# ZhaoyangLyu/Point_Diffusion_Refinement

Hardware: AMD Instinct MI355X
Metric: DDPM reverse steps/sec (T=1000, N=2048) (higher is better)
Workload: dtype f32; 1 GPU; BASELINE configs[1]: B=32/GPU, N=2048, 3072-pt mirrored condition, T=1000 DDPM reverse sampling, random-init dual-path PointNet++ (9.76 M params), cached condition step; global_batch=32, parallelism=dp1, launch=hipGraph replay, noise=device Philox, execution=fused channel-last HIP

## Files before the change

### point_diffusion_refinement_amd/csrc/abi.hip

```cpp
#include "pdr_common.h"

#include <atomic>
#include <cstring>

namespace {
thread_local char g_last_error[256] = "";

struct OptRow {
  const char* name;
  int def, lo, hi;
};
const OptRow k_opts[pdr::OPT_COUNT] = {
    {"fused_ws", 1, 0, 1},
    {"narrow_kc32", 1, 0, 1},
    {"fps_wave", 1, 0, 2},
    {"fps_lean", 1, 0, 1},
    {"knn_wave", 1, 0, 1},
    {"gn_fold_small", 1, 0, 1},
    {"ws_narrow3", 1, 0, 1},
    {"ws_xcd_order", 1, 0, 2},
    {"deep_chunks", 1, 0, 1},
    {"deep_ks", 1, 0, 1},
    {"deep_jobs32", 256, 0, 65536},
    {"deep_jobs64", 512, 0, 65536},
};
std::atomic<int> g_opts[pdr::OPT_COUNT];
std::atomic<bool> g_opts_init{false};

void opts_init() {
  if (!g_opts_init.load(std::memory_order_acquire)) {
    for (int i = 0; i < pdr::OPT_COUNT; ++i) g_opts[i].store(k_opts[i].def, std::memory_order_relaxed);
    g_opts_init.store(true, std::memory_order_release);
  }
}

int opt_index(const char* name) {
  if (!name) return -1;
  for (int i = 0; i < pdr::OPT_COUNT; ++i)
    if (std::strcmp(name, k_opts[i].name) == 0) return i;
  return -1;
}
}

namespace pdr {
void set_last_error(hipError_t e) {
  const char* s = hipGetErrorString(e);
  int i = 0;
  for (; s && s[i] && i < 255; ++i) g_last_error[i] = s[i];
  g_last_error[i] = 0;
}
int option(Opt o) {
  opts_init();
  return g_opts[o].load(std::memory_order_relaxed);
}
}

extern "C" int pdr_set_option(const char* name, int value) {
  const int i = opt_index(name);
  if (i < 0 || value < k_opts[i].lo || value > k_opts[i].hi) return PDR_EINVAL;
  opts_init();
  g_opts[i].store(value, std::memory_order_relaxed);
  return PDR_OK;
}

extern "C" int pdr_get_option(const char* name, int* value) {
  const int i = opt_index(name);
  if (i < 0 || !value) return PDR_EINVAL;
  *value = pdr::option(static_cast<pdr::Opt>(i));
  return PDR_OK;
}

extern "C" const char* pdr_option_name(int index) {
  return (index >= 0 && index < pdr::OPT_COUNT) ? k_opts[index].name : nullptr;
}

extern "C" int pdr_version(void) { return 200;  }
extern "C" const char* pdr_last_error(void) { return g_last_error; }
```

### point_diffusion_refinement_amd/csrc/fps.hip

```cpp
#include "pdr_common.h"

#include <cstdlib>

namespace {

constexpr int kMaxResidentN = 16384;

template <int T, int PPT>
__global__ __launch_bounds__(T) void fps_resident_kernel(
    const float* __restrict__ xyz, int N, int m, int R, int Rbits, int Q,
    int* __restrict__ idxs) {
  extern __shared__ __attribute__((aligned(16))) float smem[];
  constexpr int W = T / 64;
  float* sx = smem;
  float* sy = smem + N;
  float* sz = smem + 2 * N;
  unsigned long long* slots =
      reinterpret_cast<unsigned long long*>(smem + ((3 * N + 3) & ~3));

  const int b = blockIdx.x;
  const int tid = threadIdx.x;
  const float* p = xyz + static_cast<size_t>(b) * N * 3;
  int* out = idxs + static_cast<size_t>(b) * m;

  for (int i = tid; i < N; i += T) {
    sx[i] = p[i * 3 + 0];
    sy[i] = p[i * 3 + 1];
    sz[i] = p[i * 3 + 2];
  }

  float px[PPT], py[PPT], pz[PPT], tmp[PPT];
  unsigned low[PPT];
#pragma unroll
  for (int i = 0; i < PPT; ++i) {
    const int k = tid + i * T;
    if (k < N) {
      px[i] = p[k * 3 + 0];
      py[i] = p[k * 3 + 1];
      pz[i] = p[k * 3 + 2];
      const float mag = PDR_SUM3(px[i], py[i], pz[i]);
      tmp[i] = (static_cast<double>(mag) <= 1e-3) ? -1.0f : 1e10f;
      const unsigned rank = pdr::bitrev(static_cast<unsigned>(k % R), Rbits) * Q + k / R;
      low[i] = ((0xFFFFu - rank) << 16) | static_cast<unsigned>(k);
    } else {
      px[i] = py[i] = pz[i] = 0.0f;
      tmp[i] = -1.0f;
      low[i] = 0u;
    }
  }
#pragma unroll
  for (int a = 0; a < PPT - 1; ++a) {
#pragma unroll
    for (int c = 0; c < PPT - 1 - a; ++c) {
      if (low[c] < low[c + 1]) {
        float t;
        unsigned u;
        t = px[c]; px[c] = px[c + 1]; px[c + 1] = t;
        t = py[c]; py[c] = py[c + 1]; py[c + 1] = t;
        t = pz[c]; pz[c] = pz[c + 1]; pz[c + 1] = t;
        t = tmp[c]; tmp[c] = tmp[c + 1]; tmp[c + 1] = t;
        u = low[c]; low[c] = low[c + 1]; low[c + 1] = u;
      }
    }
  }

  if (tid == 0) out[0] = 0;
  __syncthreads();

  int old = 0;
  for (int j = 1; j < m; ++j) {
    const float x1 = sx[old], y1 = sy[old], z1 = sz[old];
    float best = -1.0f;
    unsigned bestlow = 0u;
#pragma unroll
    for (int i = 0; i < PPT; ++i) {
      const float dx = px[i] - x1, dy = py[i] - y1, dz = pz[i] - z1;
      const float d = PDR_SUM3(dx, dy, dz);
      const float d2 = fminf(d, tmp[i]);
      tmp[i] = d2;
      const bool gt = d2 > best;
      best = gt ? d2 : best;
      bestlow = gt ? low[i] : bestlow;
    }
    unsigned long long key =
        best < 0.0f ? 0ull : pdr::u64_from(__float_as_uint(best), bestlow);
    key = pdr::wave_max_u64(key);
    if constexpr (W > 1) {
      unsigned long long* s = slots + (j & 1) * W;
      if ((tid & 63) == 0) s[tid >> 6] = key;
      __syncthreads();
      unsigned long long r = s[0];
#pragma unroll
      for (int w = 1; w < W; ++w) {
        const unsigned long long o = s[w];
        r = o > r ? o : r;
      }
      key = r;
    }
    old = static_cast<int>(key & 0xFFFFull);
    if (tid == 0) out[j] = old;
  }
}

typedef float fps_f2 __attribute__((ext_vector_type(2)));

__device__ __forceinline__ void fps_combine(float& da, unsigned& la, float db, unsigned lb) {
  asm volatile(
      "v_cmp_gt_f32 vcc, %2, %0\n\t"
      "s_nop 1\n\t"
      "v_cndmask_b32 %0, %0, %2, vcc\n\t"
      "v_cndmask_b32 %1, %1, %3, vcc"
      : "+v"(da), "+v"(la)
      : "v"(db), "v"(lb)
      : "vcc");
}
__device__ __forceinline__ void fps_combine2(float& da, unsigned& la, float db, unsigned lb, float& dc,
                                             unsigned& lc, float dd, unsigned ld) {
  unsigned long long m;
  asm volatile(
      "v_cmp_gt_f32 vcc, %5, %0\n\t"
      "v_cmp_gt_f32 %4, %7, %2\n\t"
      "s_nop 0\n\t"
      "v_cndmask_b32 %0, %0, %5, vcc\n\t"
      "v_cndmask_b32 %1, %1, %6, vcc\n\t"
      "v_cndmask_b32 %2, %2, %7, %4\n\t"
      "v_cndmask_b32 %3, %3, %8, %4"
      : "+v"(da), "+v"(la), "+v"(dc), "+v"(lc), "=&s"(m)
      : "v"(db), "v"(lb), "v"(dd), "v"(ld)
      : "vcc");
}

template <int H>
__device__ __forceinline__ void fps_first2(const fps_f2& a, const fps_f2& b, float& bd0, unsigned& bs0, float& bd1,
                                           unsigned& bs1) {
  unsigned long long m;
  asm volatile(
      "v_cmp_gt_f32 vcc, %6, %5\n\t"
      "v_cmp_gt_f32 %4, %8, %7\n\t"
      "s_nop 0\n\t"
      "v_cndmask_b32 %0, %5, %6, vcc\n\t"
      "v_cndmask_b32 %1, %9, %10, vcc\n\t"
      "v_cndmask_b32 %2, %7, %8, %4\n\t"
      "v_cndmask_b32 %3, %11, %12, %4"
      : "=&v"(bd0), "=&v"(bs0), "=&v"(bd1), "=&v"(bs1), "=&s"(m)
      : "v"(a[0]), "v"(a[1]), "v"(b[0]), "v"(b[1]), "n"(2 * H), "n"(2 * H + 1), "n"(2 * H + 2), "n"(2 * H + 3)
      : "vcc");
}
template <int H>
__device__ __forceinline__ void fps_first1(const fps_f2& a, float& bd0, unsigned& bs0) {
  asm volatile(
      "v_cmp_gt_f32 vcc, %3, %2\n\t"
      "s_nop 1\n\t"
      "v_cndmask_b32 %0, %2, %3, vcc\n\t"
      "v_cndmask_b32 %1, %4, %5, vcc"
      : "=&v"(bd0), "=&v"(bs0)
      : "v"(a[0]), "v"(a[1]), "n"(2 * H), "n"(2 * H + 1)
      : "vcc");
}
template <int H, int NH>
__device__ __forceinline__ void fps_level0(const fps_f2 (&tmp)[NH], float (&bd)[NH], unsigned (&bs)[NH]) {
  if constexpr (H + 1 < NH) {
    fps_first2<H>(tmp[H], tmp[H + 1], bd[H], bs[H], bd[H + 1], bs[H + 1]);
    fps_level0<H + 2, NH>(tmp, bd, bs);
  } else if constexpr (H < NH) {
    fps_first1<H>(tmp[H], bd[H], bs[H]);
  }
}

template <int T, int PPT>
__global__ __launch_bounds__(T) void fps_wave_kernel(const float* __restrict__ xyz, int N, int m, int R,
                                                     int Rbits, int Q, int* __restrict__ idxs) {
  static_assert(PPT % 2 == 0, "points are processed in pairs");
  constexpr int W = T / 64;
  extern __shared__ __attribute__((aligned(16))) float4 cloud4[];
  __shared__ unsigned long long slots[2][W > 1 ? W : 1];
  const int b = blockIdx.x;
  const int lane = threadIdx.x;
  const float* p = xyz + static_cast<size_t>(b) * N * 3;
  int* out = idxs + static_cast<size_t>(b) * m;
  for (int i = lane; i < N; i += T) cloud4[i] = make_float4(p[i * 3 + 0], p[i * 3 + 1], p[i * 3 + 2], 0.0f);

  fps_f2 px[PPT / 2], py[PPT / 2], pz[PPT / 2], tmp[PPT / 2];
#pragma unroll
  for (int i = 0; i < PPT; ++i) {
    const int r = i * T + lane;
    const int hi = r / Q, lo = r - hi * Q;
    const int k = lo * R + static_cast<int>(pdr::bitrev(static_cast<unsigned>(hi), Rbits));
    const bool valid = hi < R && k < N;
    const int kk = valid ? k : 0;
    const float x = p[kk * 3 + 0], y = p[kk * 3 + 1], z = p[kk * 3 + 2];
    const float mag = PDR_SUM3(x, y, z);
    const float t0 = (!valid || static_cast<double>(mag) <= 1e-3) ? -1.0f : 1e10f;
    px[i >> 1][i & 1] = valid ? x : 0.0f;
    py[i >> 1][i & 1] = valid ? y : 0.0f;
    pz[i >> 1][i & 1] = valid ? z : 0.0f;
    tmp[i >> 1][i & 1] = t0;
  }
  if (lane == 0) out[0] = 0;
  __syncthreads();

  int old = 0;
  for (int j = 1; j < m; ++j) {
    const float4 c = cloud4[old];
    constexpr int G = (PPT / 2) < 8 ? (PPT / 2) : 8;
#pragma unroll
    for (int h0 = 0; h0 < PPT / 2; h0 += G) {
      fps_f2 dx[G], dy[G], dz[G], d[G];
#pragma unroll
      for (int g = 0; g < G; ++g) dy[g] = py[h0 + g] - c.y;
#pragma unroll
      for (int g = 0; g < G; ++g) dx[g] = px[h0 + g] - c.x;
#pragma unroll
      for (int g = 0; g < G; ++g) d[g] = dy[g] * dy[g];
#pragma unroll
      for (int g = 0; g < G; ++g) dz[g] = pz[h0 + g] - c.z;
#pragma unroll
      for (int g = 0; g < G; ++g) d[g] = __builtin_elementwise_fma(dx[g], dx[g], d[g]);
#pragma unroll
      for (int g = 0; g < G; ++g) d[g] = __builtin_elementwise_fma(dz[g], dz[g], d[g]);
#pragma unroll
      for (int g = 0; g < G; ++g) {
        fps_f2 r;
        asm("v_min_f32 %0, %1, %2" : "=v"(r[0]) : "v"(d[g][0]), "v"(tmp[h0 + g][0]));
        asm("v_min_f32 %0, %1, %2" : "=v"(r[1]) : "v"(d[g][1]), "v"(tmp[h0 + g][1]));
        tmp[h0 + g] = r;
      }
    }
    float bd[PPT / 2];
    unsigned bs[PPT / 2];
    fps_level0<0, PPT / 2>(tmp, bd, bs);
#pragma unroll
    for (int st = 1; st < PPT / 2; st <<= 1) {
#pragma unroll
      for (int i = 0; i + st < PPT / 2; i += 4 * st) {
        if (i + 3 * st < PPT / 2) fps_combine2(bd[i], bs[i], bd[i + st], bs[i + st], bd[i + 2 * st], bs[i + 2 * st],
                                               bd[i + 3 * st], bs[i + 3 * st]);
        else fps_combine(bd[i], bs[i], bd[i + st], bs[i + st]);
      }
    }
    const float best = bd[0];
    const unsigned vb = best < 0.0f ? 0u : __float_as_uint(best);
    const unsigned vmax = pdr::wave_max_u32(vb);
    const unsigned rk = 0xFFFFu - (bs[0] * static_cast<unsigned>(T) + static_cast<unsigned>(lane));
    const unsigned cand = (vb == vmax && best >= 0.0f) ? rk : 0u;
    unsigned win = pdr::wave_max_u32(cand);
    if constexpr (W > 1) {
      unsigned long long* sl = slots[j & 1];
      if ((lane & 63) == 0) sl[lane >> 6] = pdr::u64_from(vmax, win);
      __syncthreads();
      unsigned long long key = sl[0];
#pragma unroll
      for (int w = 1; w < W; ++w) {
        const unsigned long long o = sl[w];
        key = o > key ? o : key;
      }
      win = static_cast<unsigned>(key & 0xFFFFFFFFull);
    }
    const int rw = 0xFFFF - static_cast<int>(win);
    const int hw = rw / Q, lw = rw - hw * Q;
    old = win == 0u ? 0 : lw * R + static_cast<int>(pdr::bitrev(static_cast<unsigned>(hw), Rbits));
    if (lane == 0) out[j] = old;
  }
}

template <int T, int PPT>
int launch_wave(const float* xyz, int B, int N, int m, int R, int Rbits, int Q, int* idx, hipStream_t s) {
  hipLaunchKernelGGL((fps_wave_kernel<T, PPT>), dim3(B), dim3(T), static_cast<size_t>(N) * sizeof(float4), s, xyz, N,
                     m, R, Rbits, Q, idx);
  return pdr::check_launch();
}

__device__ __forceinline__ unsigned fps_wave_max_u32(unsigned v) {
  asm volatile(
      "s_nop 1\n\t"
      "v_max_u32_dpp %0, %0, %0 row_shr:1 row_mask:0xf bank_mask:0xf\n\t"
      "s_nop 1\n\t"
      "v_max_u32_dpp %0, %0, %0 row_shr:2 row_mask:0xf bank_mask:0xf\n\t"
      "s_nop 1\n\t"
      "v_max_u32_dpp %0, %0, %0 row_shr:4 row_mask:0xf bank_mask:0xf\n\t"
      "s_nop 1\n\t"
      "v_max_u32_dpp %0, %0, %0 row_shr:8 row_mask:0xf bank_mask:0xf\n\t"
      "s_nop 1\n\t"
      "v_max_u32_dpp %0, %0, %0 row_bcast:15 row_mask:0xa bank_mask:0xf\n\t"
      "s_nop 1\n\t"
      "v_max_u32_dpp %0, %0, %0 row_bcast:31 row_mask:0xc bank_mask:0xf\n\t"
      "s_nop 1"
      : "+v"(v));
  return __builtin_amdgcn_readlane(v, 63);
}

template <int T, int PPT>
__global__ __launch_bounds__(T) void fps_lean_kernel(const float* __restrict__ xyz, int N, int m, int R, int Rbits,
                                                     int Q, int* __restrict__ idxs) {
  static_assert(PPT % 2 == 0, "points are updated in pairs");
  constexpr int W = T / 64;
  extern __shared__ __attribute__((aligned(16))) float4 lean_cloud[];
  __shared__ unsigned long long slots[2][W > 1 ? W : 1];
  const int b = blockIdx.x;
  const int tid = threadIdx.x;
  const float* p = xyz + static_cast<size_t>(b) * N * 3;
  int* out = idxs + static_cast<size_t>(b) * m;
  for (int i = tid; i < N; i += T) lean_cloud[i] = make_float4(p[i * 3 + 0], p[i * 3 + 1], p[i * 3 + 2], 0.0f);

  float sx[PPT], sy[PPT], sz[PPT], st[PPT];
  unsigned low[PPT];
#pragma unroll
  for (int i = 0; i < PPT; ++i) {
    const int k = tid + i * T;
    if (k < N) {
      sx[i] = p[k * 3 + 0];
      sy[i] = p[k * 3 + 1];
      sz[i] = p[k * 3 + 2];
      const float mag = PDR_SUM3(sx[i], sy[i], sz[i]);
      st[i] = (static_cast<double>(mag) <= 1e-3) ? -1.0f : 1e10f;
      const unsigned rank = pdr::bitrev(static_cast<unsigned>(k % R), Rbits) * Q + k / R;
      low[i] = ((0xFFFFu - rank) << 16) | static_cast<unsigned>(k);
    } else {
      sx[i] = sy[i] = sz[i] = 0.0f;
      st[i] = -1.0f;
      low[i] = 0u;
    }
  }
#pragma unroll
  for (int a = 0; a < PPT - 1; ++a) {
#pragma unroll
    for (int c = 0; c < PPT - 1 - a; ++c) {
      if (low[c] < low[c + 1]) {
        float t;
        unsigned u;
        t = sx[c]; sx[c] = sx[c + 1]; sx[c + 1] = t;
        t = sy[c]; sy[c] = sy[c + 1]; sy[c + 1] = t;
        t = sz[c]; sz[c] = sz[c + 1]; sz[c + 1] = t;
        t = st[c]; st[c] = st[c + 1]; st[c + 1] = t;
        u = low[c]; low[c] = low[c + 1]; low[c + 1] = u;
      }
    }
  }
  fps_f2 px[PPT / 2], py[PPT / 2], pz[PPT / 2], tmp[PPT / 2];
#pragma unroll
  for (int i = 0; i < PPT; ++i) {
    px[i >> 1][i & 1] = sx[i];
    py[i >> 1][i & 1] = sy[i];
    pz[i >> 1][i & 1] = sz[i];
    tmp[i >> 1][i & 1] = st[i];
  }
  if (tid == 0) out[0] = 0;
  __syncthreads();

  int old = 0;
  for (int j = 1; j < m; ++j) {
    const float4 c = lean_cloud[old];
    constexpr int G = PPT / 2;
    fps_f2 dx[G], dy[G], dz[G], d[G];
#pragma unroll
    for (int g = 0; g < G; ++g) dy[g] = py[g] - c.y;
#pragma unroll
    for (int g = 0; g < G; ++g) dx[g] = px[g] - c.x;
#pragma unroll
    for (int g = 0; g < G; ++g) d[g] = dy[g] * dy[g];
#pragma unroll
    for (int g = 0; g < G; ++g) dz[g] = pz[g] - c.z;
#pragma unroll
    for (int g = 0; g < G; ++g) d[g] = __builtin_elementwise_fma(dx[g], dx[g], d[g]);
#pragma unroll
    for (int g = 0; g < G; ++g) d[g] = __builtin_elementwise_fma(dz[g], dz[g], d[g]);
    float best = -1.0f;
    unsigned bestlow = 0u;
#pragma unroll
    for (int g = 0; g < G; ++g) {
      fps_f2 r;
      asm("v_min_f32 %0, %1, %2" : "=v"(r[0]) : "v"(d[g][0]), "v"(tmp[g][0]));
      asm("v_min_f32 %0, %1, %2" : "=v"(r[1]) : "v"(d[g][1]), "v"(tmp[g][1]));
      tmp[g] = r;
#pragma unroll
      for (int e = 0; e < 2; ++e) {
        const bool gt = r[e] > best;
        best = gt ? r[e] : best;
        bestlow = gt ? low[2 * g + e] : bestlow;
      }
    }
    const unsigned vb = best < 0.0f ? 0u : __float_as_uint(best);
    const unsigned vmax = fps_wave_max_u32(vb);
    const unsigned cand = (vb == vmax && !(best < 0.0f)) ? bestlow : 0u;
    unsigned wlow = fps_wave_max_u32(cand);
    unsigned long long key = pdr::u64_from(vmax, wlow);
    if constexpr (W > 1) {
      unsigned long long* sl = slots[j & 1];
      if ((tid & 63) == 0) sl[tid >> 6] = key;
      __syncthreads();
      unsigned long long r = sl[0];
#pragma unroll
      for (int w = 1; w < W; ++w) {
        const unsigned long long o = sl[w];
        r = o > r ? o : r;
      }
      key = r;
    }
    old = static_cast<int>(key & 0xFFFFull);
    if (tid == 0) out[j] = old;
  }
}

template <int T, int PPT>
int launch_lean(const float* xyz, int B, int N, int m, int R, int Rbits, int Q, int* idx, hipStream_t s) {
  hipLaunchKernelGGL((fps_lean_kernel<T, PPT>), dim3(B), dim3(T), static_cast<size_t>(N) * sizeof(float4), s, xyz, N, m,
                     R, Rbits, Q, idx);
  return pdr::check_launch();
}

__global__ __launch_bounds__(1024) void fps_stream_kernel(
    const float* __restrict__ xyz, int N, int m, int R, int Rbits, int Q,
    float* __restrict__ temp, int* __restrict__ idxs) {
  __shared__ float sval[16];
  __shared__ unsigned long long srank[16];
  __shared__ int sold;
  const int b = blockIdx.x, tid = threadIdx.x;
  const float* p = xyz + static_cast<size_t>(b) * N * 3;
  float* tp = temp + static_cast<size_t>(b) * N;
  int* out = idxs + static_cast<size_t>(b) * m;
  for (int k = tid; k < N; k += 1024) {
    const float mag = PDR_SUM3(p[k * 3], p[k * 3 + 1], p[k * 3 + 2]);
    tp[k] = (static_cast<double>(mag) <= 1e-3) ? -1.0f : 1e10f;
  }
  if (tid == 0) out[0] = 0;
  __syncthreads();
  int old = 0;
  for (int j = 1; j < m; ++j) {
    const float x1 = p[old * 3], y1 = p[old * 3 + 1], z1 = p[old * 3 + 2];
    float best = -1.0f;
    unsigned long long bestrank = ~0ull;
    for (int k = tid; k < N; k += 1024) {
      const float dx = p[k * 3] - x1, dy = p[k * 3 + 1] - y1, dz = p[k * 3 + 2] - z1;
      const float d2 = fminf(PDR_SUM3(dx, dy, dz), tp[k]);
      tp[k] = d2;
      const unsigned long long rank =
          (static_cast<unsigned long long>(pdr::bitrev(k % R, Rbits)) * Q + k / R) << 32 |
          static_cast<unsigned>(k);
      const bool better = d2 > best || (d2 == best && d2 >= 0.0f && rank < bestrank);
      best = better ? d2 : best;
      bestrank = better ? rank : bestrank;
    }
#pragma unroll
    for (int off = 32; off >= 1; off >>= 1) {
      const float ov = __shfl_xor(best, off, 64);
      const unsigned long long orank = __shfl_xor(bestrank, off, 64);
      const bool better = ov > best || (ov == best && orank < bestrank);
      best = better ? ov : best;
      bestrank = better ? orank : bestrank;
    }
    if ((tid & 63) == 0) {
      sval[tid >> 6] = best;
      srank[tid >> 6] = bestrank;
    }
    __syncthreads();
    if (tid == 0) {
      float bv = sval[0];
      unsigned long long br = srank[0];
      for (int w = 1; w < 16; ++w) {
        const bool better = sval[w] > bv || (sval[w] == bv && srank[w] < br);
        bv = better ? sval[w] : bv;
        br = better ? srank[w] : br;
      }
      sold = bv < 0.0f ? 0 : static_cast<int>(br & 0xFFFFFFFFull);
      out[j] = sold;
    }
    __syncthreads();
    old = sold;
  }
}

template <int T, int PPT>
int launch_resident(const float* xyz, int B, int N, int m, int R, int Rbits, int Q,
                    int* idx, hipStream_t s) {
  const size_t lds = static_cast<size_t>((3 * N + 3) & ~3) * sizeof(float) +
                     2 * (T / 64) * sizeof(unsigned long long);
  if (lds > 64 * 1024 &&
      hipFuncSetAttribute(reinterpret_cast<const void*>(&fps_resident_kernel<T, PPT>),
                          hipFuncAttributeMaxDynamicSharedMemorySize, 160 * 1024) != hipSuccess)
    return PDR_ELAUNCH;
  hipLaunchKernelGGL((fps_resident_kernel<T, PPT>), dim3(B), dim3(T), lds, s, xyz, N, m, R,
                     Rbits, Q, idx);
  return pdr::check_launch();
}

}

extern "C" int pdr_opt_n_threads(int work_size) {
  if (work_size <= 0) return 1;
  const int pow_2 = static_cast<int>(log(static_cast<double>(work_size)) / log(2.0));
  int t = 1 << pow_2;
  if (t > 512) t = 512;
  if (t < 1) t = 1;
  return t;
}

extern "C" size_t pdr_fps_workspace_bytes(int B, int N) {
  if (B <= 0 || N <= 0) return 0;
  return (N <= 12288) ? 0 : static_cast<size_t>(B) * N * sizeof(float);
}

extern "C" int pdr_furthest_point_sampling(const float* xyz, int B, int N, int m,
                                           float* temp, int* idx, pdr_stream_t stream) {
  if (B < 0 || N <= 0 || m < 0) return PDR_EINVAL;
  if (B == 0 || m == 0) return PDR_OK;
  if (!xyz || !idx) return PDR_EINVAL;
  hipStream_t s = pdr::as_stream(stream);
  const int R = pdr_opt_n_threads(N);
  int Rbits = 0;
  while ((1 << Rbits) < R) ++Rbits;
  const int Q = (N + R - 1) / R;
  if (pdr_fps_workspace_bytes(B, N) > 0) {
    if (!temp) return PDR_EINVAL;
    hipLaunchKernelGGL(fps_stream_kernel, dim3(B), dim3(1024), 0, s, xyz, N, m, R, Rbits, Q,
                       temp, idx);
    return pdr::check_launch();
  }
  const int wave_mode = pdr::option(pdr::OPT_FPS_WAVE);
  const bool use_wave = wave_mode == 2 || (wave_mode == 1 && static_cast<long>(R) * Q <= 256);
  const bool wave_fits = static_cast<size_t>(N) * sizeof(float4) + 256 <= 64 * 1024;
  if (use_wave && wave_fits && static_cast<long>(R) * Q <= 4096) {
    const long slots = static_cast<long>(R) * Q;
    if (slots <= 128) return launch_wave<64, 2>(xyz, B, N, m, R, Rbits, Q, idx, s);
    if (slots <= 256) return launch_wave<64, 4>(xyz, B, N, m, R, Rbits, Q, idx, s);
    if (slots <= 512) return launch_wave<256, 2>(xyz, B, N, m, R, Rbits, Q, idx, s);
    if (slots <= 1024) return launch_wave<256, 4>(xyz, B, N, m, R, Rbits, Q, idx, s);
    if (slots <= 2048) return launch_wave<256, 8>(xyz, B, N, m, R, Rbits, Q, idx, s);
    return launch_wave<256, 16>(xyz, B, N, m, R, Rbits, Q, idx, s);
  }
  const bool lean = pdr::option(pdr::OPT_FPS_LEAN) != 0;
  if (lean && N > 128 && static_cast<size_t>(N) * sizeof(float4) + 256 <= 64 * 1024) {
    if (N <= 512) return launch_lean<256, 2>(xyz, B, N, m, R, Rbits, Q, idx, s);
    if (N <= 1024) return launch_lean<256, 4>(xyz, B, N, m, R, Rbits, Q, idx, s);
    if (N <= 2048) return launch_lean<256, 8>(xyz, B, N, m, R, Rbits, Q, idx, s);
    if (N <= 3072) return launch_lean<256, 12>(xyz, B, N, m, R, Rbits, Q, idx, s);
    return launch_lean<256, 16>(xyz, B, N, m, R, Rbits, Q, idx, s);
  }
  static_assert(kMaxResidentN >= 12288, "resident path must cover the LDS-resident range");
#define PDR_FPS_CASE(T, PPT) \
  if (N <= (T) * (PPT)) return launch_resident<T, PPT>(xyz, B, N, m, R, Rbits, Q, idx, s)
  PDR_FPS_CASE(64, 1);
  PDR_FPS_CASE(64, 2);
  PDR_FPS_CASE(256, 1);
  PDR_FPS_CASE(256, 2);
  PDR_FPS_CASE(256, 4);
  PDR_FPS_CASE(256, 8);
  PDR_FPS_CASE(256, 12);
  PDR_FPS_CASE(256, 16);
  PDR_FPS_CASE(1024, 8);
  PDR_FPS_CASE(1024, 12);
#undef PDR_FPS_CASE
  return PDR_EUNSUPPORTED;
}
```

Baseline: 5996 cloud-steps/s.

## Add register-resident FPS chain kernel carrying winner coordinates through reductions

Adds a new farthest-point-sampling kernel that keeps each thread's points in registers, sorted by tie-break rank, and uses inline-asm compare/select pairs for the per-thread argmax. The winning point's coordinates travel with the key through the wave and block reductions, so the next centroid does not need a dependent LDS load each iteration. It becomes the default for fps_lean=1, and the previous lean kernel moves to mode 2. This targets the serial per-iteration latency of FPS, at the cost of hand-written asm with hazard nops and more register pressure.

```diff
diff --git a/point_diffusion_refinement_amd/csrc/abi.hip b/point_diffusion_refinement_amd/csrc/abi.hip
--- a/point_diffusion_refinement_amd/csrc/abi.hip
+++ b/point_diffusion_refinement_amd/csrc/abi.hip
@@ -14,7 +14,7 @@
     {"fused_ws", 1, 0, 1},
     {"narrow_kc32", 1, 0, 1},
     {"fps_wave", 1, 0, 2},
-    {"fps_lean", 1, 0, 1},
+    {"fps_lean", 1, 0, 2},
     {"knn_wave", 1, 0, 1},
     {"gn_fold_small", 1, 0, 1},
     {"ws_narrow3", 1, 0, 1},
diff --git a/point_diffusion_refinement_amd/csrc/fps.hip b/point_diffusion_refinement_amd/csrc/fps.hip
--- a/point_diffusion_refinement_amd/csrc/fps.hip
+++ b/point_diffusion_refinement_amd/csrc/fps.hip
@@ -405,6 +405,207 @@
 int launch_lean(const float* xyz, int B, int N, int m, int R, int Rbits, int Q, int* idx, hipStream_t s) {
   hipLaunchKernelGGL((fps_lean_kernel<T, PPT>), dim3(B), dim3(T), static_cast<size_t>(N) * sizeof(float4), s, xyz, N, m,
                      R, Rbits, Q, idx);
+  return pdr::check_launch();
+}
+
+
+__device__ __forceinline__ void fps_pair2(float a, unsigned la, float b, unsigned lb, float c, unsigned lc, float d,
+                                          unsigned ld, float& o0, unsigned& p0, float& o1, unsigned& p1) {
+  unsigned long long msk;
+  asm volatile(
+      "v_cmp_gt_f32 vcc, %6, %5\n\t"
+      "v_cmp_gt_f32 %4, %10, %9\n\t"
+      "s_nop 0\n\t"
+      "v_cndmask_b32 %0, %5, %6, vcc\n\t"
+      "v_cndmask_b32 %1, %7, %8, vcc\n\t"
+      "v_cndmask_b32 %2, %9, %10, %4\n\t"
+      "v_cndmask_b32 %3, %11, %12, %4"
+      : "=&v"(o0), "=&v"(p0), "=&v"(o1), "=&v"(p1), "=&s"(msk)
+      : "v"(a), "v"(b), "v"(la), "v"(lb), "v"(c), "v"(d), "v"(lc), "v"(ld)
+      : "vcc");
+}
+__device__ __forceinline__ void fps_pair1(float a, unsigned la, float b, unsigned lb, float& o0, unsigned& p0) {
+  asm volatile(
+      "v_cmp_gt_f32 vcc, %3, %2\n\t"
+      "s_nop 1\n\t"
+      "v_cndmask_b32 %0, %2, %3, vcc\n\t"
+      "v_cndmask_b32 %1, %4, %5, vcc"
+      : "=&v"(o0), "=&v"(p0)
+      : "v"(a), "v"(b), "v"(la), "v"(lb)
+      : "vcc");
+}
+
+struct alignas(16) FpsRecord {
+  unsigned lo, hi;
+  float x, y;
+  float z, pad0, pad1, pad2;
+};
+
+template <int T, int PPT, bool kBallot, bool kCarry>
+__global__ __launch_bounds__(T) void fps_chain_kernel(const float* __restrict__ xyz, int N, int m, int R, int Rbits,
+                                                      int Q, int* __restrict__ idxs) {
+  static_assert(PPT % 2 == 0, "points are updated in pairs");
+  constexpr int W = T / 64;
+  constexpr int NP = PPT / 2;
+  extern __shared__ __attribute__((aligned(16))) float4 chain_cloud[];
+  __shared__ FpsRecord recs[2][W];
+  const int b = blockIdx.x;
+  const int tid = threadIdx.x;
+  const int lane = tid & 63;
+  const float* p = xyz + static_cast<size_t>(b) * N * 3;
+  int* out = idxs + static_cast<size_t>(b) * m;
+  for (int i = tid; i < N; i += T) chain_cloud[i] = make_float4(p[i * 3 + 0], p[i * 3 + 1], p[i * 3 + 2], 0.0f);
+
+  float sx[PPT], sy[PPT], sz[PPT], st[PPT];
+  unsigned low[PPT];
+#pragma unroll
+  for (int i = 0; i < PPT; ++i) {
+    const int k = tid + i * T;
+    if (k < N) {
+      sx[i] = p[k * 3 + 0];
+      sy[i] = p[k * 3 + 1];
+      sz[i] = p[k * 3 + 2];
+      const float mag = PDR_SUM3(sx[i], sy[i], sz[i]);
+      st[i] = (static_cast<double>(mag) <= 1e-3) ? -1.0f : 1e10f;
+      const unsigned rank = pdr::bitrev(static_cast<unsigned>(k % R), Rbits) * Q + k / R;
+      low[i] = ((0xFFFFu - rank) << 16) | static_cast<unsigned>(k);
+    } else {
+      sx[i] = sy[i] = sz[i] = 0.0f;
+      st[i] = -1.0f;
+      low[i] = 0u;
+    }
+  }
+#pragma unroll
+  for (int a = 0; a < PPT - 1; ++a) {
+#pragma unroll
+    for (int c = 0; c < PPT - 1 - a; ++c) {
+      if (low[c] < low[c + 1]) {
+        float t;
+        unsigned u;
+        t = sx[c]; sx[c] = sx[c + 1]; sx[c + 1] = t;
+        t = sy[c]; sy[c] = sy[c + 1]; sy[c + 1] = t;
+        t = sz[c]; sz[c] = sz[c + 1]; sz[c + 1] = t;
+        t = st[c]; st[c] = st[c + 1]; st[c + 1] = t;
+        u = low[c]; low[c] = low[c + 1]; low[c + 1] = u;
+      }
+    }
+  }
+  fps_f2 px[NP], py[NP], pz[NP], tmp[NP];
+#pragma unroll
+  for (int i = 0; i < PPT; ++i) {
+    px[i >> 1][i & 1] = sx[i];
+    py[i >> 1][i & 1] = sy[i];
+    pz[i >> 1][i & 1] = sz[i];
+    tmp[i >> 1][i & 1] = st[i];
+  }
+  if (tid == 0) out[0] = 0;
+  float cx = p[0], cy = p[1], cz = p[2];
+  __syncthreads();
+
+  int old = 0;
+  for (int j = 1; j < m; ++j) {
+    if constexpr (!kCarry) {
+      const float4 c = chain_cloud[old];
+      cx = c.x; cy = c.y; cz = c.z;
+    }
+    fps_f2 dx[NP], dy[NP], dz[NP], d[NP];
+#pragma unroll
+    for (int g = 0; g < NP; ++g) dy[g] = py[g] - cy;
+#pragma unroll
+    for (int g = 0; g < NP; ++g) dx[g] = px[g] - cx;
+#pragma unroll
+    for (int g = 0; g < NP; ++g) d[g] = dy[g] * dy[g];
+#pragma unroll
+    for (int g = 0; g < NP; ++g) dz[g] = pz[g] - cz;
+#pragma unroll
+    for (int g = 0; g < NP; ++g) d[g] = __builtin_elementwise_fma(dx[g], dx[g], d[g]);
+#pragma unroll
+    for (int g = 0; g < NP; ++g) d[g] = __builtin_elementwise_fma(dz[g], dz[g], d[g]);
+#pragma unroll
+    for (int g = 0; g < NP; ++g) {
+      fps_f2 r;
+      asm("v_min_f32 %0, %1, %2" : "=v"(r[0]) : "v"(d[g][0]), "v"(tmp[g][0]));
+      asm("v_min_f32 %0, %1, %2" : "=v"(r[1]) : "v"(d[g][1]), "v"(tmp[g][1]));
+      tmp[g] = r;
+    }
+    float bd[NP];
+    unsigned bl[NP];
+#pragma unroll
+    for (int g = 0; g + 1 < NP; g += 2)
+      fps_pair2(tmp[g][0], low[2 * g], tmp[g][1], low[2 * g + 1], tmp[g + 1][0], low[2 * g + 2], tmp[g + 1][1],
+                low[2 * g + 3], bd[g], bl[g], bd[g + 1], bl[g + 1]);
+    if constexpr (NP % 2 == 1)
+      fps_pair1(tmp[NP - 1][0], low[PPT - 2], tmp[NP - 1][1], low[PPT - 1], bd[NP - 1], bl[NP - 1]);
+#pragma unroll
+    for (int s2 = 1; s2 < NP; s2 <<= 1) {
+#pragma unroll
+      for (int i = 0; i + s2 < NP; i += 4 * s2) {
+        if (i + 3 * s2 < NP) fps_combine2(bd[i], bl[i], bd[i + s2], bl[i + s2], bd[i + 2 * s2], bl[i + 2 * s2],
+                                          bd[i + 3 * s2], bl[i + 3 * s2]);
+        else fps_combine(bd[i], bl[i], bd[i + s2], bl[i + s2]);
+      }
+    }
+    const float best = bd[0];
+    const unsigned bestlow = bl[0];
+    const float4 own = kCarry ? chain_cloud[bestlow & 0xFFFFu] : make_float4(0.f, 0.f, 0.f, 0.f);
+    const unsigned vb1 = best < 0.0f ? 0u : __float_as_uint(best) + 1u;
+    const unsigned vmax1 = fps_wave_max_u32(vb1);
+    const unsigned vmax = vmax1 == 0u ? 0u : vmax1 - 1u;
+    const unsigned long long holders = __builtin_amdgcn_ballot_w64(vb1 == vmax1);
+    unsigned wlow = 0u;
+    int wl = 0;
+    if (!kBallot) {
+      const unsigned cand = (vmax1 != 0u && vb1 == vmax1) ? bestlow : 0u;
+      wlow = fps_wave_max_u32(cand);
+      if (kCarry) wl = __builtin_ctzll(__builtin_amdgcn_ballot_w64(cand == wlow) | (1ull << 63));
+    } else if (vmax1 != 0u) {
+      if ((holders & (holders - 1ull)) == 0ull) {
+        wl = __builtin_ctzll(holders);
+      } else {
+        const unsigned cand = ((holders >> lane) & 1ull) ? bestlow : 0u;
+        const unsigned wmax = fps_wave_max_u32(cand);
+        wl = __builtin_ctzll(__builtin_amdgcn_ballot_w64(cand == wmax));
+      }
+      wlow = __builtin_amdgcn_readlane(bestlow, wl);
+    }
+    unsigned klo = wlow, khi = vmax;
+    float nx = __uint_as_float(__builtin_amdgcn_readlane(__float_as_uint(own.x), wl));
+    float ny = __uint_as_float(__builtin_amdgcn_readlane(__float_as_uint(own.y), wl));
+    float nz = __uint_as_float(__builtin_amdgcn_readlane(__float_as_uint(own.z), wl));
+    if constexpr (W > 1) {
+      FpsRecord* rs = recs[j & 1];
+      if (lane == 0) {
+        FpsRecord r;
+        r.lo = klo; r.hi = khi; r.x = nx; r.y = ny;
+        r.z = nz; r.pad0 = r.pad1 = r.pad2 = 0.0f;
+        rs[tid >> 6] = r;
+      }
+      __syncthreads();
+      FpsRecord r0 = rs[0];
+      klo = r0.lo; khi = r0.hi; nx = r0.x; ny = r0.y; nz = r0.z;
+#pragma unroll
+      for (int w = 1; w < W; ++w) {
+        const FpsRecord o = rs[w];
+        const bool gt = pdr::u64_from(o.hi, o.lo) > pdr::u64_from(khi, klo);
+        klo = gt ? o.lo : klo;
+        khi = gt ? o.hi : khi;
+        nx = gt ? o.x : nx;
+        ny = gt ? o.y : ny;
+        nz = gt ? o.z : nz;
+      }
+    }
+    cx = nx;
+    cy = ny;
+    cz = nz;
+    old = static_cast<int>(klo & 0xFFFFu);
+    if (tid == 0) out[j] = old;
+  }
+}
+
+template <int T, int PPT, bool kBallot = true, bool kCarry = true>
+int launch_chain(const float* xyz, int B, int N, int m, int R, int Rbits, int Q, int* idx, hipStream_t s) {
+  hipLaunchKernelGGL((fps_chain_kernel<T, PPT, kBallot, kCarry>), dim3(B), dim3(T), static_cast<size_t>(N) * sizeof(float4), s, xyz, N,
+                     m, R, Rbits, Q, idx);
   return pdr::check_launch();
 }
 
@@ -527,8 +728,16 @@
     if (slots <= 2048) return launch_wave<256, 8>(xyz, B, N, m, R, Rbits, Q, idx, s);
     return launch_wave<256, 16>(xyz, B, N, m, R, Rbits, Q, idx, s);
   }
-  const bool lean = pdr::option(pdr::OPT_FPS_LEAN) != 0;
-  if (lean && N > 128 && static_cast<size_t>(N) * sizeof(float4) + 256 <= 64 * 1024) {
+  const int lean_mode = pdr::option(pdr::OPT_FPS_LEAN);
+  const bool fits = N > 128 && static_cast<size_t>(N) * sizeof(float4) + 256 <= 64 * 1024;
+  if (lean_mode == 1 && fits) {
+    if (N <= 512) return launch_chain<256, 2>(xyz, B, N, m, R, Rbits, Q, idx, s);
+    if (N <= 1024) return launch_chain<256, 4>(xyz, B, N, m, R, Rbits, Q, idx, s);
+    if (N <= 2048) return launch_chain<256, 8>(xyz, B, N, m, R, Rbits, Q, idx, s);
+    if (N <= 3072) return launch_chain<256, 12>(xyz, B, N, m, R, Rbits, Q, idx, s);
+    return launch_chain<256, 16>(xyz, B, N, m, R, Rbits, Q, idx, s);
+  }
+  if (lean_mode == 2 && fits) {
     if (N <= 512) return launch_lean<256, 2>(xyz, B, N, m, R, Rbits, Q, idx, s);
     if (N <= 1024) return launch_lean<256, 4>(xyz, B, N, m, R, Rbits, Q, idx, s);
     if (N <= 2048) return launch_lean<256, 8>(xyz, B, N, m, R, Rbits, Q, idx, s);
```

Result: slower. 5873 cloud-steps/s (median of 2 runs) (-2.1%).
